# ethereum/pos-evolution

Hardware: AMD Instinct MI355X
Metric: attestations aggregated/sec + get_head() p50 latency at 1M validators (higher is better)
Workload: dtype int32

## Files before the change

pos_evolution_amd/csrc/att_bodies.inc:

```
#include <algorithm>
#include "att_row.h"
#include "kernels.h"
#include "wave64.h"

namespace posevo {

namespace {

constexpr uint32_t VAL_EQUIVOCATING_BIT = 0x04u;
constexpr uint32_t FLAG_SIG_VALID = 0x1u, FLAG_FROM_BLOCK = 0x2u, FLAG_OVERLAPPING = 0x4u;
constexpr int32_t ST_OK = 0, ST_EPOCH_TIME = 1, ST_EPOCH_SLOT = 2, ST_UNKNOWN_TARGET = 3, ST_UNKNOWN_BLOCK = 4,
                  ST_BLOCK_AFTER_SLOT = 5, ST_TARGET_NOT_ANCESTOR = 6, ST_SLOT_NOT_PAST = 7, ST_NO_TABLE = 8,
                  ST_INDEX_RANGE = 9, ST_BITS_LENGTH = 10, ST_EMPTY = 11, ST_BAD_SIGNATURE = 12, ST_INCLUSION = 13,
                  ST_SOURCE = 14;
constexpr uint32_t ERR_INVALID_ARG = 1, ERR_CAPACITY = 10, ERR_NO_COMMITTEES = 11;

struct Row9 { uint4 q[9]; };
__device__ __forceinline__ void load_row(Row9& r, const uint4* __restrict__ rows, uint32_t i)
{
    const uint4* p = rows + (size_t)9 * i;
#pragma unroll
    for (int k = 0; k < 9; ++k) r.q[k] = p[k];
}
__device__ __forceinline__ unsigned long long u64_of(uint32_t lo, uint32_t hi) { return ((unsigned long long)hi << 32) | lo; }
// ... 422 lines not shown
{
    uint32_t h = r0.x & bt.root_mask;
    for (;;) {
        const uint32_t idx = bt.root_tab[h];
        if (idx == NONE32) return NONE32;
        const uint4* q = reinterpret_cast<const uint4*>(bt.roots + 32ull * idx);
        if (same4(q[0], r0) && same4(q[1], r1)) return idx;
        h = (h + 1) & bt.root_mask;
    }
}
}

namespace {
__device__ __forceinline__ void att_validate_fc_body(const uint32_t g , const ValidateFcArgs& a)
{
    const uint4* __restrict__ rows = static_cast<const uint4*>(a.rows);
    const AttGroup* __restrict__ grp = a.grp;
    const AttPlan* __restrict__ plan = a.plan;
    const uint32_t cap = a.cap;
    const BlockTableDev& bt = a.bt;
    const FcCtx& fc = a.fc;
    const uint32_t* __restrict__ union_info = a.union_info;
    AttRow* __restrict__ out_rows = a.out_rows;
    int32_t* __restrict__ status_dev = a.status_dev;
    int32_t* __restrict__ status_host = a.status_host;
    uint32_t* __restrict__ count_host = a.count_host;
    uint32_t* __restrict__ err_host = a.err_host;
    const uint32_t ng = plan->n_groups;
    if (ng > cap) {
        if (g < ng) status_dev[g] = -1;
        if (g == 0) *err_host = ERR_CAPACITY;
        return;
    }
    if (g >= ng) return;
    const AttGroup G = grp[g];
    Row9 r;
    load_row(r, rows, G.rep);
    const unsigned long long slot = row_slot(r), tep = row_target_epoch(r), spe = fc.slots_per_epoch;
    const uint32_t flags = r.q[8].z;
    int32_t st = ST_OK;
    uint32_t blk = NONE32;
    if (!(flags & FLAG_FROM_BLOCK) && tep != fc.cur_epoch && tep != fc.prev_epoch) st = ST_EPOCH_TIME;
    else if (tep != slot / spe) st = ST_EPOCH_SLOT;
    else {
        const uint32_t tgt = find_block_dev(bt, r.q[6], r.q[7]);
        if (tgt == NONE32) st = ST_UNKNOWN_TARGET;
        else {
            blk = find_block_dev(bt, r.q[1], r.q[2]);
            if (blk == NONE32) st = ST_UNKNOWN_BLOCK;
            else {
                uint32_t p = bt.pos_of_idx[blk];
                if (bt.slot_pos[p] > slot) st = ST_BLOCK_AFTER_SLOT;
                else {
                    const unsigned long long start = tep * spe;
                    while (bt.slot_pos[p] > start && bt.parent_pos[p] != NONE32) p = bt.parent_pos[p];
                    if (p != bt.pos_of_idx[tgt]) st = ST_TARGET_NOT_ANCESTOR;
                    else if (fc.cur_slot < slot + 1) st = ST_SLOT_NOT_PAST;
                }
            }
        }
    }
    if (st == ST_OK && G.status_agg) st = (int32_t)G.status_agg;
    const uint32_t cnt = union_info[2 * g], overlap = union_info[2 * g + 1];
    if (st == ST_OK) {
        if (!G.sig_valid) st = ST_BAD_SIGNATURE;
        else if (overlap) st = ST_BAD_SIGNATURE;
        else if (cnt == 0) st = ST_EMPTY;
    }
    AttRow o;
    o.member_base = G.member_base;
    o.n_bits = G.size;
    o.bits_word = G.out_word;
    o.block_idx = blk;
    o.epoch_p1 = (uint32_t)tep + 1;
    o.order = g;
    o.flag_mask = 0;
    o.which = 0;
    o.slot = (uint32_t)slot;
    o.gate = g;
    out_rows[g] = o;
    status_dev[g] = st;
    status_host[g] = st;
    if (count_host) count_host[g] = st == ST_OK ? cnt : 0u;
}
}

namespace {
__device__ __forceinline__ void lmd_vm_tables_body(const unsigned long long v , const LmdVmArgs& a)
{
    const AttRow* __restrict__ rows = a.rows;
    const TablesDev& tables = a.tables;
    const uint32_t* __restrict__ cs0 = a.crow_start[0];
    const uint32_t* __restrict__ cs1 = a.crow_start[1];
    const uint32_t* __restrict__ cl0 = a.crow_list[0];
    const uint32_t* __restrict__ cl1 = a.crow_list[1];
    const AttPlan* __restrict__ plan = a.plan;
    const uint32_t* __restrict__ bit_arena = a.bit_arena;
    const uint8_t* __restrict__ flags = a.flags;
    unsigned long long* __restrict__ vote_key = reinterpret_cast<unsigned long long*>(a.vote_key);
    uint32_t* __restrict__ vote_block = a.vote_block;
    uint32_t* __restrict__ vote_slot = a.vote_slot;
    const uint32_t* __restrict__ gates = a.gates;
    if (v >= a.n_val) return;
    uint32_t best_e = 0, best_order = NONE32, new_block = NONE32, new_slot = 0;
    bool loaded = false;
    for (int t = 0; t < 2; ++t) {
        if (!tables.t[t].valid || plan->n_rows_table[t] == 0) continue;
        const uint32_t c = tables.t[t].inv_comm[v];
        if (c == NONE32) continue;
        const uint32_t* crow_start = t ? cs1 : cs0;
        const uint32_t* crow_list = t ? cl1 : cl0;
        const uint32_t kb = crow_start[c], ke = crow_start[c + 1];
        if (kb == ke) continue;
        if (!loaded) {
            if (flags[v] & VAL_EQUIVOCATING_BIT) return;
            best_e = (uint32_t)(vote_key[v] >> 32);
            loaded = true;
        }
        const uint32_t i = tables.t[t].inv_pos[v];
        for (uint32_t k = kb; k < ke; ++k) {
            const AttRow r = rows[crow_list[k]];
            if (i >= r.n_bits) continue;
            if (gates[r.gate] != 0) continue;
            if (!((bit_arena[r.bits_word + (i >> 5)] >> (i & 31)) & 1u)) continue;
            if (r.epoch_p1 > best_e || (r.epoch_p1 == best_e && new_block != NONE32 && r.order < best_order)) {
                best_e = r.epoch_p1;
                best_order = r.order;
                new_block = r.block_idx;
                new_slot = r.slot;
            }
        }
    }
    if (new_block != NONE32) {
        vote_key[v] = ((unsigned long long)best_e << 32) | 0xFFFFFFFFull;
        vote_block[v] = new_block;
        if (vote_slot) vote_slot[v] = new_slot;
    }
}
}

}
```

pos_evolution_amd/csrc/engine_internal.h:

```cpp
#pragma once
#include <hip/hip_runtime.h>
#include <dlfcn.h>
#include <rccl/rccl.h>

#include <algorithm>
#include <array>
#include <chrono>
#include <cstdlib>
#include <map>
#include <cstdio>
#include <cstddef>
#include <cstring>
#include <functional>
#include <memory>
#include <new>
#include <numeric>
#include <string>
#include <thread>
#include <unordered_map>
#include <vector>

#include "../../include/posevo.h"
#include "../../include/posevo_profile.h"
#include "att_row.h"
// ... 285 lines not shown
        hipEvent_t ev_leg = nullptr;
        bool leg_used = false;
        bool fenced = false, side_used = false, aux_used = false;
        bool fence_pending = false;
        bool aux_reads_scratch = false;
    };
    static constexpr int MAX_ARENAS = 16;
    int n_arenas = 3;
    PipeArena arena[MAX_ARENAS];
    int cur = 0;
    PipeArena& A() { return arena[cur]; }
    bool pipelining = false;
    uint64_t pipes_begun = 0, pipes_completed = 0;
    hipStream_t side_stream = nullptr;
    uint64_t arena_growths = 0;
    bool queues_distinct = false;
    hipStream_t fin_stream = nullptr;
    hipStream_t norm_stream = nullptr;
    hipEvent_t ev_tree = nullptr;
    hipStream_t g1_tail() const { return norm_stream ? norm_stream : fin_stream; }
    hipStream_t aux_stream = nullptr;
    hipStream_t aux_owned = nullptr;
    hipStream_t prep_stream = nullptr;
    DevBuf d_shuffle_scratch;
    hipStream_t sums_stream = nullptr;
    DevBuf d_sum_groups, d_sum_lane;
    uint32_t last_cmpl_groups = 0;
    hipEvent_t ev_aux_fork = nullptr;
    hipEvent_t ev_aux_switch = nullptr;
    static constexpr uint32_t STATE_ON_SIDE_MAX_ROWS = 1024;
    bool aux_busy = false;
    bool state_work_on_main = false;
    hipEvent_t ev_acc = nullptr;
    struct SigSeg {
        int arena;
        uint32_t n;
        bool compressed, check_subgroup;
        bool streaming;
        const uint8_t* d_in;
        const uint8_t* copy_from;
        size_t bytes;
        uint32_t* d_pts; int32_t* d_status;
        const UnionGroup* d_ug; const uint32_t* d_member_row; uint32_t ng_bound; const AttPlan* plan_dev;
        uint8_t* o_sig; uint32_t* o_bad; int32_t* o_st;
        uint32_t* keep_mont48; uint32_t* keep_bad;
    };
    std::vector<SigSeg> sig_batch;
    hipEvent_t ev_sig = nullptr;
    hipEvent_t ev_fork = nullptr, ev_join = nullptr;
    bool side_busy = false;
    bool side_ever = false;
    bool streaming = false;
    std::vector<std::function<int()>> deferred;
    struct HeldFc {
        bool active = false;
        int arena = -1;
        bool have_fc = false;
        bool have_head = false;
        ValidateFcArgs validate{};
        LmdVmArgs lmd{};
        VotesArgs votes{};
        TreeArgs tree{};
        std::function<int()> between;
        std::vector<std::function<int()>> g1;
        bool fence_pending = false;
    } held;
    bool pairing = std::getenv("POSEVO_PAIR") == nullptr || std::atoi(std::getenv("POSEVO_PAIR")) != 0;
    struct Tune {
        static int env(const char* name, int dflt)
        {
            const char* e = std::getenv(name);
            return e && *e ? std::atoi(e) : dflt;
        }
        int exclusive = env("POSEVO_ACC_EXCLUSIVE", 1);
        int state_on = env("POSEVO_STATE_ON", 2);
        int sig_batch = env("POSEVO_SIG_BATCH", 8);
        int queue_probe = env("POSEVO_QUEUE_PROBE", 1);
        int committee_sums = env("POSEVO_COMMITTEE_SUMS", 1);
        int g1_sparse = env("POSEVO_G1_SPARSE", 1);
        uint32_t g1_sparse_max() const
        {
            return g1_sparse <= 0 ? 0u : g1_sparse == 1 ? G1_SPARSE_MAX : std::min<uint32_t>((uint32_t)g1_sparse, G1_SPARSE_CAP);
        }
        uint32_t ssz_tile_log2 = (uint32_t)std::min<int>(SSZ_TILE_LOG2, std::max<int>(SSZ_TILE_LOG2_MIN, env("POSEVO_SSZ_TILE_LOG2", SSZ_TILE_LOG2)));
    } tune;

    struct ResGroup { uint32_t byte_off, n_bits, word, sig_valid, tag; };
    std::vector<ResGroup> res_groups;
    std::shared_ptr<std::vector<uint32_t>> res_info_host;
    bool res_valid = false;
    int res_arena = 0;
    uint64_t res_generation = 0;

    struct ResidentRows {
        bool valid = false;
        int arena = 0;
        uint32_t n_in = 0;
        const void* rows = nullptr;
        TablesDev tables{};
        uint64_t generation = 0;
        int set = 0;
        uint32_t n_groups = 0;
    } rr;

    int g1_tune_calls = 0;
    float g1_tune_best[2] = {1e30f, 1e30f};
    uint32_t g1_target_slots = 0;
    hipEvent_t g1_tune_ev[2] = {nullptr, nullptr};
    bool points30_valid = false;
    DevBuf d_points30, d_tmp_points30;

    ncclComm_t comm = nullptr, comm_g1 = nullptr;
    int early_rc = PE_OK;
    uint32_t xchg_blocks = 0;
    uint64_t xchg_nval = 0;
    bool last_agg_on_side = false;
    int dist_rank = 0, dist_world = 1;
    DevBuf d_xchg, d_xpart, d_xgather;
    pe_collectives coll{};
    bool coll_custom = false;
    bool dist_single_comm = false;
    bool dist_wedged = false;
    uint32_t dist_timeout_ms = 30000;
    uint32_t dist_max_groups = 0;
    hipEvent_t ev_xchg = nullptr;
    bool dist_ready() const { return comm != nullptr || coll_custom; }

    struct Slasher {
        bool enabled = false;
        uint32_t history = 0, max_data = 0;
        uint64_t n_val = 0;
        bool have_window = false;
        uint64_t window = 0;
        DevBuf d_rec, d_ids, d_counter, d_evidence;
        struct EpochData {
            std::vector<std::array<uint8_t, 128>> data;
            std::unordered_map<std::string, uint32_t> id_of;
        };
        std::vector<EpochData> epochs;
        bool on_device = false;
        uint32_t tab_size = 0;
        DevBuf d_data, d_count, d_tab;
        DevBuf d_work;
        std::vector<uint32_t> dev_count;
    } slasher;

    bool profiling = false;
    uint64_t acc_launches = 0;
    static constexpr uint32_t ACC_CLOCK_RING = 4096;
    unsigned long long* acc_clock = nullptr;
    uint64_t acc_clock_n = 0;
    KernelProfile prof[PE_KERNEL_COUNT];
    bool prof_timeline = false;
    bool prof_dominant_only = false;
    hipEvent_t prof_base = nullptr;
    struct TimelineEntry { int32_t kernel; float start_ms, dur_ms; };
    std::vector<TimelineEntry> prof_tl;
    std::vector<hipEvent_t> event_pool;
    HostTrace trace;
};

namespace posevo {

int fail(pe_engine* h, int code, const std::string& msg);
int hip_fail(pe_engine* h, hipError_t e, const char* what);
#define HIP_TRY(h, expr)                                        \
// ... 408 lines not shown
```

pos_evolution_amd/csrc/engine_resident.cpp:

```cpp
#include "engine_internal.h"


using namespace posevo;

namespace posevo {

namespace {

struct RrLayout {
    AttPlan* plan;
    uint32_t *slot_of, *rep_of, *gid_of_row, *ubytes, *member_row;
    PlanSync* sync;
    PlanRec* rec;
    AttGroup* grp;
    UnionGroup* ug;
    G1Group* g1;
    AttRow *rows_fc, *rows_st;
    int32_t *status_fc, *status_st;
    uint32_t* cmpl;
    uint32_t *crow_start[2], *crow_cursor[2], *crow_cnt[2], *crow_list[2];
    size_t bytes;
};

RrLayout rr_layout(uint8_t* base, uint32_t cap_n, uint32_t cap_c)
{
    RrLayout L;
    size_t off = 0;
    auto take = [&](size_t bytes) {
        uint8_t* p = base ? base + off : nullptr;
        off = (off + bytes + 255) & ~size_t(255);
        return p;
    };
    L.plan = reinterpret_cast<AttPlan*>(take(sizeof(AttPlan)));
    L.slot_of = reinterpret_cast<uint32_t*>(take(4ull * cap_n));
    L.rep_of = reinterpret_cast<uint32_t*>(take(4ull * cap_n));
    L.gid_of_row = reinterpret_cast<uint32_t*>(take(4ull * cap_n));
    L.sync = reinterpret_cast<PlanSync*>(take(sizeof(PlanSync)));
    L.rec = reinterpret_cast<PlanRec*>(take(sizeof(PlanRec) * ((size_t)cap_n / PLAN_WG + 1)));
    L.ubytes = reinterpret_cast<uint32_t*>(take(4ull * cap_n));
    L.member_row = reinterpret_cast<uint32_t*>(take(4ull * cap_n));
    L.grp = reinterpret_cast<AttGroup*>(take(sizeof(AttGroup) * (size_t)cap_n));
    L.ug = reinterpret_cast<UnionGroup*>(take(sizeof(UnionGroup) * (size_t)cap_n));
    L.g1 = reinterpret_cast<G1Group*>(take(sizeof(G1Group) * (size_t)cap_n));
    L.rows_fc = reinterpret_cast<AttRow*>(take(sizeof(AttRow) * (size_t)cap_n));
    L.rows_st = reinterpret_cast<AttRow*>(take(sizeof(AttRow) * (size_t)cap_n));
    L.status_fc = reinterpret_cast<int32_t*>(take(4ull * cap_n));
    L.status_st = reinterpret_cast<int32_t*>(take(4ull * cap_n));
    L.cmpl = reinterpret_cast<uint32_t*>(take(4ull * cap_n));
    for (int t = 0; t < 2; ++t) {
        L.crow_start[t] = reinterpret_cast<uint32_t*>(take(4ull * (cap_c + 1)));
        L.crow_cursor[t] = reinterpret_cast<uint32_t*>(take(4ull * (cap_c + 1)));
        L.crow_cnt[t] = reinterpret_cast<uint32_t*>(take(4ull * (cap_c + 1)));
        L.crow_list[t] = reinterpret_cast<uint32_t*>(take(4ull * cap_n));
    }
    L.bytes = off;
    return L;
}

struct RrSet {
    DevBuf &tab, &rr, &bits, &info;
    uint32_t &rows_cap, &comm_cap, &tab_size;
};
RrSet rr_set(pe_engine::PipeArena& a, int set)
{
    if (set == 0) return RrSet{a.d_rr_tab, a.d_rr, a.d_res_bits, a.d_res_info, a.rr_rows_cap, a.rr_comm_cap, a.rr_tab_size};
    return RrSet{a.x_rr_tab, a.x_rr, a.x_res_bits, a.x_res_info, a.x_rows_cap, a.x_comm_cap, a.x_tab_size};
}
RrLayout rr_of(pe_engine::PipeArena& a, int set = 0)
{
    const RrSet s = rr_set(a, set);
    return rr_layout(s.rr.as<uint8_t>(), s.rows_cap, s.comm_cap);
}

int rr_ensure(pe_engine* h, pe_engine::PipeArena& arena, int set, uint32_t n, uint32_t n_comm)
{
    {
        const RrSet rs = rr_set(arena, set);
        if (n <= rs.rows_cap && n_comm <= rs.comm_cap && rs.rr.p && rs.tab.p) return PE_OK;
    }
    PE_TRY(flush_pending(h));
    HIP_TRY(h, hipDeviceSynchronize());
    uint32_t cap_n = 1024, cap_c = 64;
    for (int i = 0; i < h->n_arenas; ++i) {
        const RrSet o = rr_set(h->arena[i], set);
        cap_n = std::max(cap_n, o.rows_cap);
        cap_c = std::max(cap_c, o.comm_cap);
    }
    while (cap_n < n) cap_n *= 2;
    while (cap_c < n_comm) cap_c *= 2;
    uint32_t tab = 2048;
    while (tab < 2 * cap_n) tab <<= 1;
    const RrLayout L = rr_layout(nullptr, cap_n, cap_c);
    for (int i = 0; i < h->n_arenas; ++i) {
        pe_engine::PipeArena& other = h->arena[i];
        if (set != 0 && &other != &arena) continue;
        const RrSet a = rr_set(other, set);
        if (cap_n <= a.rows_cap && cap_c <= a.comm_cap && a.rr.p && a.tab.p) continue;
        a.rr.release();
        a.tab.release();
        HIP_TRY(h, a.rr.ensure(L.bytes));
        HIP_TRY(h, a.tab.ensure(8ull * tab));
        HIP_TRY(h, hipMemsetAsync(a.tab.p, 0xFF, 4ull * tab, h->stream));
        HIP_TRY(h, hipMemsetAsync(a.tab.as<uint8_t>() + 4ull * tab, 0, 4ull * tab, h->stream));
        HIP_TRY(h, hipMemsetAsync(a.rr.p, 0, L.bytes, h->stream));
        a.rows_cap = cap_n;
        a.comm_cap = cap_c;
        a.tab_size = tab;
    }
    HIP_TRY(h, hipStreamSynchronize(h->stream));
    return PE_OK;
}

int candidate_tables(pe_engine* h, TablesDev* out, CommitteeTable* tabs[2])
{
    memset(out, 0, sizeof(*out));
    out->slots_per_epoch = h->cfg.slots_per_epoch;
    const uint64_t cur = epoch_at_slot(h, current_slot(h));
    const uint64_t prev = cur > 0 ? cur - 1 : cur;
    const uint64_t epochs[2] = {cur, prev};
    for (int k = 0; k < 2; ++k) {
        tabs[k] = nullptr;
        out->t[k].epoch = epochs[k];
        if (k == 1 && prev == cur) continue;
        CommitteeTable* t = find_table(h, epochs[k]);
        if (!t) continue;
        if (!t->is_partition || t->n_val_at_load != h->n_val || !t->d_inv_comm.p)
            return fail(h, PE_ERR_INVALID_ARG,
                        "rows in device memory: the committee tables of the current / previous epoch must partition the "
                        "registry they were loaded for (use host rows otherwise)");
        tabs[k] = t;
        out->t[k].members = t->d_members.as<uint32_t>();
        out->t[k].offsets = t->d_offsets.as<uint32_t>();
        out->t[k].inv_comm = t->d_inv_comm.as<uint32_t>();
        out->t[k].inv_pos = t->d_inv_pos.as<uint32_t>();
        out->t[k].n_committees = t->n_committees;
        out->t[k].valid = 1;
    }
    return PE_OK;
}

uint32_t g1_target_slots(const pe_engine* h)
{
    if (h->streaming) return G1_TARGET_LANES / 2;
    return h->g1_target_slots ? h->g1_target_slots : G1_TARGET_LANES;
}

}

int plan_error_to_status(pe_engine* h, uint32_t err, const char* who)
{
    switch (err) {
        case 0: return PE_OK;
        case 10: return fail(h, PE_ERR_CAPACITY, std::string(who) + ": output capacity too small for the groups formed");
        case 11: return fail(h, PE_ERR_NO_COMMITTEES, std::string(who) + ": no committee table for a group's target epoch");
        case 12: return fail(h, PE_ERR_NO_DEVICE, std::string(who) + ": a workgroup of k_att_plan gave up waiting for its predecessors' records");
        default:
            return fail(h, PE_ERR_INVALID_ARG, std::string(who) + ": a row was refused on the device (bits exceed the arena, "
                        "target epoch beyond 32 bits, committee index out of range or len(aggregation_bits) != len(committee))");
    }
}

MemKind mem_kind(const void* p)
{
    hipPointerAttribute_t pa;
    if (p && hipPointerGetAttributes(&pa, p) == hipSuccess)
        return pa.type == hipMemoryTypeDevice ? MemKind::Device : pa.type == hipMemoryTypeHost ? MemKind::Pinned : MemKind::Pageable;
    (void)hipGetLastError();
    return MemKind::Pageable;
}
bool rows_on_device(const void* p) { return p && p != (const void*)PE_ROWS_RESIDENT && mem_kind(p) == MemKind::Device; }

BlockTableDev block_table_dev(const pe_engine* h)
{
    BlockTableDev bt;
    bt.root_tab = h->d_broot_tab.as<uint32_t>();
    bt.root_mask = h->broot_mask;
    bt.roots = h->d_broots.as<uint8_t>();
    bt.slot_pos = h->d_bslot_pos.as<unsigned long long>();
    bt.parent_pos = h->d_tparent.as<uint32_t>();
    bt.pos_of_idx = h->d_tpos.as<uint32_t>();
    bt.n_blocks = (uint32_t)h->blocks.size();
    return bt;
}

int aggregate_resident(pe_engine* h, const pe_attestation* d_rows, uint32_t n, const uint8_t* bits_arena,
                       uint64_t arena_len, pe_attestation* out_atts, uint32_t* out_n_groups, uint32_t* group_of,
                       uint8_t* out_bits_arena, uint64_t out_arena_cap, uint8_t* out_aggpk96, uint32_t* out_count,
                       uint32_t* dev_partials, int set, const uint32_t* n_dev)
{
    if (!h->initialised) return fail(h, PE_ERR_STATE, "rows in device memory: the store's clock picks the committee tables; call pe_store_init first");
    if ((uintptr_t)d_rows & 15) return fail(h, PE_ERR_INVALID_ARG, "rows in device memory must be 16-byte aligned");
    if (arena_len >= 0xFFFFFFF0ull) return fail(h, PE_ERR_CAPACITY, "bit arena exceeds 4 GiB");
    if (n >= PLAN_MAX_ROWS) return fail(h, PE_ERR_CAPACITY, "rows in device memory: at most 2^24 - 1 rows per aggregate");
    const bool want_pk = out_aggpk96 != nullptr || dev_partials != nullptr;
    if (want_pk && !h->have_points) return fail(h, PE_ERR_STATE, "aggregate pubkeys requested but no pubkeys loaded");
    HostLap lap(&h->trace);
    TablesDev tables;
    CommitteeTable* tabs[2];
    PE_TRY(candidate_tables(h, &tables, tabs));
    const uint32_t n_comm = std::max(tables.t[0].n_committees, tables.t[1].n_committees);
    pe_engine::PipeArena& A = h->A();
    PE_TRY(rr_ensure(h, A, set, n, n_comm));
    const RrLayout L = rr_of(A, set);
    const RrSet RS = rr_set(A, set);
    const uint32_t target = g1_target_slots(h);
    const uint32_t slot_cap = std::max<uint32_t>(2 * G1_TARGET_LANES, (n + G1_WG - 1) / G1_WG * G1_WG);
    const size_t words_cap = (size_t)out_arena_cap / 4 + n + 16;
    Stage st(h);
    PE_TRY(st.reserve((size_t)arena_len + 256));
    const size_t pad_at = ((size_t)arena_len + 15) & ~size_t(15);
    const size_t off_arena = st.alloc(pad_at + 32);
    if (set == 0) {
        PE_TRY(ensure_quiesced_arenas(h, &pe_engine::PipeArena::d_res_bits, words_cap * 4 + 64));
        PE_TRY(ensure_quiesced_arenas(h, &pe_engine::PipeArena::d_res_info, 8ull * n + 64));
    } else {
        PE_TRY(ensure_quiesced(h, RS.bits, words_cap * 4 + 64));
        PE_TRY(ensure_quiesced(h, RS.info, 8ull * n + 64));
    }
    OutBlock ob(h);
    const size_t off_plan = ob.alloc(sizeof(AttPlan));
    const size_t off_rows = ob.alloc(sizeof(pe_attestation) * (size_t)n);
    const size_t off_gof = ob.alloc(4ull * n);
    const size_t off_obits = ob.alloc(words_cap * 4);
    const size_t off_oinfo = ob.alloc(8ull * n);
    const size_t off_opk = out_aggpk96 ? ob.alloc(96ull * n) : 0;
    G1Complement cm;
    bool by_cmpl = false;
    if (out_aggpk96 && !dev_partials && set == 0 && h->tune.committee_sums && !h->dist_ready())
        for (int t = 0; t < 2; ++t) {
            if (tabs[t]) PE_TRY(committee_sums_build_wanted(h, tabs[t]));
            if (tabs[t] && tabs[t]->sums_valid && tabs[t]->d_sums.p && tabs[t]->ev_sums) {
                cm.sums[t] = tabs[t]->d_sums.as<uint32_t>();
                cm.ev[t] = tabs[t]->ev_sums;
                by_cmpl = true;
            }
        }
    const size_t off_ocm = by_cmpl ? ob.alloc(4ull * n) : 0;
    PE_TRY(ob.ensure());
    if (by_cmpl) {
        cm.cmpl = L.cmpl;
        cm.info = RS.info.as<uint32_t>();
    }
    if (want_pk) {
        PE_TRY(ensure_quiesced_arenas(h, &pe_engine::PipeArena::d_partials, std::max<size_t>(PE_G1_PARTIAL_BYTES, (size_t)PE_G1_PARTIAL_BYTES * n)));
        PE_TRY(ensure_quiesced_arenas(h, &pe_engine::PipeArena::d_lane_partials, (size_t)G1_LANE_PARTIAL_BYTES * slot_cap));
        PE_TRY(ensure_quiesced(h, h->d_partials, std::max<size_t>(PE_G1_PARTIAL_BYTES, (size_t)PE_G1_PARTIAL_BYTES * n)));
        PE_TRY(ensure_quiesced(h, h->d_lane_partials, (size_t)G1_LANE_PARTIAL_BYTES * slot_cap));
    }
    lap.mark("ragg.1_reserve");
    *out_n_groups = 0;
    AttPlan* plan_host = ob.host<AttPlan>(off_plan);
    memset(plan_host, 0, sizeof(AttPlan));
    plan_host->error = 0xFFFFFFFFu;
    const MemKind arena_kind = arena_len ? mem_kind(bits_arena) : MemKind::Pageable;
    hipStream_t ms = h->stream;
    const bool pair_ok = h->held.active && h->held.arena != h->cur && set == 0 && !n_dev && hold_eligible(h);
    if (h->held.active && !pair_ok) PE_TRY(held_issue(h));
    if (set == 0) {
        if (!h->deferred.empty()) PE_TRY(run_deferred(h));
        if (A.side_used) HIP_TRY(h, hipStreamWaitEvent(ms, h->ev_join, 0));
        if (sig_batch_holds(h, h->cur)) PE_TRY(sig_batch_flush(h));
        if (A.leg_used) HIP_TRY(h, hipStreamWaitEvent(ms, A.ev_leg, 0));
        PE_TRY(aux_join(h, ms));
    }
    h->res_valid = false;
    h->rr.valid = false;
    const size_t deferred_before = h->deferred.size();
    struct Unwind {
        pe_engine* h; size_t keep; bool armed = true;
        ~Unwind() { if (armed) { h->rr.valid = false; if (h->deferred.size() > keep) h->deferred.resize(keep); } }
    } unwind{h, deferred_before};
    bool ingest_copies = false;
    if (arena_kind == MemKind::Pageable) {
        memcpy(st.host<uint8_t>(off_arena), bits_arena, arena_len);
        memset(st.host<uint8_t>(off_arena) + arena_len, 0, pad_at + 32 - arena_len);
        HIP_TRY(h, st.upload());
    } else if (arena_len) {
        if (arena_kind == MemKind::Device && (reinterpret_cast<uintptr_t>(bits_arena) & 15) == 0 && n > 0) ingest_copies = true;
        else HIP_TRY(h, hipMemcpyAsync(st.dev<uint8_t>(off_arena), bits_arena, arena_len,
                                       arena_kind == MemKind::Device ? hipMemcpyDeviceToDevice : hipMemcpyHostToDevice, ms));
    }
    lap.mark("ragg.2_bits");
    uint32_t* cnt_tab = RS.tab.as<uint32_t>() + RS.tab_size;
    const IngestArgs ia{d_rows, n, RS.tab.as<uint32_t>(), cnt_tab, RS.tab_size - 1, L.slot_of, arena_len, L.plan,
                        st.dev<uint8_t>(off_arena) + pad_at, n_dev, ingest_copies ? bits_arena : nullptr,
// ... 116 lines not shown
        if (out_aggpk96) memcpy(out_aggpk96, pin + off_opk, 96ull * ng);
        h->last_cmpl_groups = 0;
        if (by_cmpl) {
            const uint32_t* ocm = reinterpret_cast<const uint32_t*>(pin + off_ocm);
            for (uint32_t g = 0; g < ng; ++g) h->last_cmpl_groups += ocm[g] != NONE32 ? 1u : 0u;
        }
        return PE_OK;
    };
    HostLap lap2(&h->trace);
    const int rc = finish_call(h, st, ob, complete);
    lap2.mark("ragg.5_wait_outputs");
    return rc;
}

int resident_plan_dev(pe_engine* h, const AttPlan** out)
{
    if (!h->rr.valid) return fail(h, PE_ERR_STATE, "no aggregate over rows in device memory on this handle");
    *out = rr_of(h->arena[h->rr.arena], h->rr.set).plan;
    return PE_OK;
}

int resident_parts(pe_engine* h, ResidentParts* out)
{
    if (!h->rr.valid) return fail(h, PE_ERR_STATE, "no aggregate over rows in device memory on this handle");
    pe_engine::PipeArena& RA = h->arena[h->rr.arena];
    const RrLayout L = rr_of(RA, h->rr.set);
    const RrSet RS = rr_set(RA, h->rr.set);
    out->rows = h->rr.rows;
    out->grp = L.grp;
    out->plan = L.plan;
    out->res_bits = RS.bits.as<uint32_t>();
    out->res_info = RS.info.as<uint32_t>();
    out->n_in = h->rr.n_in;
    return PE_OK;
}

int resident_lists(pe_engine* h, const UnionGroup** ug, const uint32_t** member_row)
{
    if (!h->rr.valid) return fail(h, PE_ERR_STATE, "no aggregate over rows in device memory on this handle");
    const RrLayout L = rr_of(h->arena[h->rr.arena], h->rr.set);
    *ug = L.ug;
    *member_row = L.member_row;
    return PE_OK;
}

int resident_precheck(pe_engine* h, const char* who)
{
    if (!h->rr.valid) return fail(h, PE_ERR_STATE, std::string(who) + ": PE_ROWS_RESIDENT without a pe_aggregate over rows in device memory on this handle");
    TablesDev now;
    CommitteeTable* tabs[2];
    PE_TRY(candidate_tables(h, &now, tabs));
    for (int t = 0; t < 2; ++t)
        if (now.t[t].epoch != h->rr.tables.t[t].epoch || now.t[t].valid != h->rr.tables.t[t].valid ||
            now.t[t].members != h->rr.tables.t[t].members)
            return fail(h, PE_ERR_STATE, std::string(who) + ": the store's clock or its committee tables changed since the resident pe_aggregate: aggregate again");
    return PE_OK;
}

int on_attestation_resident(pe_engine* h, uint32_t cap, int32_t* status, uint32_t* out_count)
{
    PE_TRY(resident_precheck(h, "pe_on_attestation_batch"));
    if (cap == 0) return PE_OK;
    if (h->held.active && (h->held.arena != h->cur || h->held.have_fc || h->held.have_head)) PE_TRY(held_issue(h));
    HostLap lap(&h->trace);
    PE_TRY(refresh_tree(h));
    pe_engine::PipeArena& RA = h->arena[h->rr.arena];
    const RrLayout L = rr_of(RA, h->rr.set);
    const RrSet RS = rr_set(RA, h->rr.set);
    Stage st(h);
    OutBlock ob(h);
    const size_t off_status = ob.alloc(4ull * cap);
    const size_t off_count = ob.alloc(4ull * cap);
    const size_t off_err = ob.alloc(16);
    PE_TRY(ob.ensure());
    *ob.host<uint32_t>(off_err) = 0;
    FcCtx fc;
    fc.cur_slot = current_slot(h);
    fc.cur_epoch = epoch_at_slot(h, fc.cur_slot);
    fc.prev_epoch = fc.cur_epoch > 0 ? fc.cur_epoch - 1 : 0;
    fc.slots_per_epoch = h->cfg.slots_per_epoch;
    const uint32_t n_launch = std::max<uint32_t>(h->rr.n_in, 1);
    memset(ob.host<int32_t>(off_status), 0, 4ull * cap);
    memset(ob.host<uint32_t>(off_count), 0, 4ull * cap);
    const ValidateFcArgs va{h->rr.rows, L.grp, L.plan, n_launch, cap, block_table_dev(h), fc, RS.info.as<uint32_t>(), L.rows_fc,
                            L.status_fc, ob.host<int32_t>(off_status), ob.host<uint32_t>(off_count), ob.host<uint32_t>(off_err)};
    const LmdVmArgs la{L.rows_fc, h->rr.tables, {L.crow_start[0], L.crow_start[1]}, {L.crow_list[0], L.crow_list[1]}, L.plan,
                       RS.bits.as<uint32_t>(), h->d_flags.as<uint8_t>(), h->n_val, h->d_vote_key.as<uint64_t>(),
                       h->d_vote_block.as<uint32_t>(), h->cfg.vote_expiry_slots ? h->d_vote_slot.as<uint32_t>() : nullptr,
                       reinterpret_cast<const uint32_t*>(L.status_fc)};
    if (hold_eligible(h) && h->rr.arena == h->cur && h->rr.set == 0 && h->n_val) {
        h->held.validate = va;
        h->held.lmd = la;
        h->held.have_fc = true;
        h->held.active = true;
        h->held.arena = h->cur;
    } else {
        if (h->held.active) PE_TRY(held_issue(h));
        {
            ProfScope ps(h, PE_KERNEL_ATT_VALIDATE);
            launch_att_validate_fc(h->stream, va);
        }
        ProfScope ps(h, PE_KERNEL_LMD);
        launch_lmd_vm_tables(h->stream, la);
    }
    HIP_TRY(h, hipGetLastError());
    lap.mark("ratt.1_launch");
    const size_t base = ob.base;
    const int ai = h->cur;
    auto complete = [h, ai, base, off_status, off_count, off_err, cap, status, out_count]() -> int {
        const uint8_t* pin = h->arena[ai].h_pin.as<uint8_t>() + base;
        const uint32_t err = *reinterpret_cast<const uint32_t*>(pin + off_err);
        if (err) return plan_error_to_status(h, err, "pe_on_attestation_batch (PE_ROWS_RESIDENT)");
        memcpy(status, pin + off_status, 4ull * cap);
        if (out_count) memcpy(out_count, pin + off_count, 4ull * cap);
        return PE_OK;
    };
    HostLap lap2(&h->trace);
    const int rc = finish_call(h, st, ob, complete);
    lap2.mark("ratt.2_wait_outputs");
    return rc;
}

int process_attestation_resident(pe_engine* h, const pe_state_ctx* sc, uint32_t cap, int32_t* status, uint64_t* out_numerators)
{
    PE_TRY(resident_precheck(h, "pe_process_attestation_batch"));
    if (cap == 0) return PE_OK;
    const uint64_t spe = h->cfg.slots_per_epoch;
    if (spe > 64) return fail(h, PE_ERR_CAPACITY, "PE_ROWS_RESIDENT: SLOTS_PER_EPOCH above 64");
    uint32_t tip;
    if (!find_block(h, to_root(sc->chain_tip_root), &tip)) return fail(h, PE_ERR_UNKNOWN_ROOT, "chain tip unknown");
    HostLap lap(&h->trace);
    PE_TRY(refresh_tree(h));
    pe_engine::PipeArena& RA = h->arena[h->rr.arena];
    const RrLayout L = rr_of(RA, h->rr.set);
    const RrSet RS = rr_set(RA, h->rr.set);
    Stage st(h);
    StateCtxDev S;
    memset(&S, 0, sizeof(S));
    S.slot = sc->slot;
    S.cur_epoch = sc->slot / spe;
    S.prev_epoch = S.cur_epoch > 0 ? S.cur_epoch - 1 : 0;
    S.slots_per_epoch = spe;
    S.min_inclusion_delay = h->cfg.min_attestation_inclusion_delay;
    S.sqrt_spe = isqrt64(spe);
    S.cj_epoch = sc->current_justified_epoch;
    S.pj_epoch = sc->previous_justified_epoch;
    memcpy(S.cj_root, sc->current_justified_root, 32);
    memcpy(S.pj_root, sc->previous_justified_root, 32);
    S.base_reward_per_increment = sc->base_reward_per_increment;
    {
        uint32_t cur = tip;
        for (uint64_t j = spe; j-- > 0;) {
            if (S.slot + j < spe) { S.head_blk[j] = NONE32; continue; }
            cur = get_ancestor(h, cur, S.slot + j - spe);
            S.head_blk[j] = cur;
        }
        S.tgt_blk[0] = get_ancestor(h, tip, S.cur_epoch * spe);
        S.tgt_blk[1] = get_ancestor(h, tip, S.prev_epoch * spe);
    }
    OutBlock ob(h);
    const size_t off_err = ob.alloc(16);
    const size_t off_status = ob.alloc(4ull * cap);
    const size_t off_num = ob.alloc(8ull * cap);
    PE_TRY(ob.ensure());
    *ob.host<uint32_t>(off_err) = 0;
    memset(ob.host<int32_t>(off_status), 0, 4ull * cap);
    memset(ob.host<uint64_t>(off_num), 0, 8ull * cap);
    const uint32_t n_launch = std::max<uint32_t>(h->rr.n_in, 1);
    hipStream_t ss = state_stream_begin(h, true, n_launch);
    {
        ProfScope ps(h, PE_KERNEL_ATT_VALIDATE, ss);
        launch_att_validate_state(ss, h->rr.rows, L.grp, L.plan, n_launch, cap, block_table_dev(h), S,
// ... 30 lines not shown
```

pos_evolution_amd/csrc/kernels.h:

```cpp
#pragma once
#include <hip/hip_runtime.h>
#include <stdint.h>

namespace posevo {

template <int TAG>
static bool first_use_on_this_device()
{
    static bool done[64] = {false};
    int dev = 0;
    (void)hipGetDevice(&dev);
    if (dev < 0 || dev >= 64) return true;
    if (done[dev]) return false;
    done[dev] = true;
    return true;
}

constexpr uint32_t NONE32 = 0xFFFFFFFFu;
constexpr int G1_ROW_WORDS = 32;
constexpr int G2_WG_SLOTS = 128;
constexpr int G1_WG = 256;
constexpr int G1_LANE_PARTIAL_BYTES = 208;
constexpr int TREE_MAX_BLOCKS = 8192;
constexpr int VOTES_MAX_WG = 256;
// ... 107 lines not shown
    uint32_t last_error;
    unsigned long long total_members;
};
struct AttGroup {
    uint32_t rep;
    uint32_t n_atts, list_start, cursor;
    uint32_t n_bits, out_word, out_byte;
    uint32_t table;
    uint32_t pos, size, member_base;
    uint32_t sig_valid;
    uint32_t status_agg;
    uint32_t index_over;
    uint32_t pad[2];
};
struct BlockTableDev {
    const uint32_t* root_tab;
    uint32_t root_mask;
    const uint8_t* roots;
    const unsigned long long* slot_pos;
    const uint32_t* parent_pos;
    const uint32_t* pos_of_idx;
    uint32_t n_blocks;
};
struct FcCtx {
    unsigned long long cur_slot, cur_epoch, prev_epoch, slots_per_epoch;
};
struct StateCtxDev {
    unsigned long long slot, cur_epoch, prev_epoch, slots_per_epoch, min_inclusion_delay, sqrt_spe;
    unsigned long long cj_epoch, pj_epoch;
    uint8_t cj_root[32], pj_root[32];
    uint32_t tgt_blk[2];
    uint32_t head_blk[64];
    unsigned long long base_reward_per_increment;
};
struct PlanSync {
    uint32_t ticket;
    uint32_t max_size;
    uint32_t rows_t[2];
    uint32_t mis_key;
    uint32_t err;
    uint32_t pad[2];
    unsigned long long total_members, pad2[3];
};
struct PlanRec {
    unsigned long long agg[3], incl[3], pad[2];
};
constexpr uint32_t PLAN_WG = 256;
constexpr uint32_t PLAN_MAX_ROWS = 1u << 24;
struct AttPlanArgs {
    const void* rows; uint32_t n; const uint32_t* n_dev;
    const uint32_t* tab; const uint32_t* cnt_tab; const uint32_t* slot_of;
    uint32_t* rep_of; uint32_t* gid_of_row;
    AttGroup* grp; UnionGroup* ug;
    uint32_t* crow_start[2]; uint32_t* crow_cursor[2]; uint32_t* crow_cnt[2];
    PlanSync* sync; PlanRec* rec;
    AttPlan* plan; AttPlan* plan_host;
    uint64_t out_arena_cap; uint32_t target_slots, slot_cap, min_k, want_pk;
    TablesDev tables;
};
void launch_att_plan(hipStream_t s, const AttPlanArgs& a);
void launch_att_pack(hipStream_t s, const void* rows, const AttGroup* grp, const AttPlan* plan, const uint32_t* res_bits,
                     const uint32_t* res_info, uint32_t slots, uint32_t wps, uint32_t* send);
void launch_att_unpack(hipStream_t s, const uint32_t* recv, uint32_t world, uint32_t slots, uint32_t wps, void* out_rows,
                       uint32_t* out_bits, uint32_t* n_dev, uint32_t* err_host);
void launch_att_validate_state(hipStream_t s, const void* rows, const AttGroup* grp, const AttPlan* plan, uint32_t n_bound,
                               uint32_t cap, BlockTableDev bt, const StateCtxDev& st, const uint32_t* union_info,
                               AttRow* out_rows, int32_t* status_dev, int32_t* status_host, uint32_t* err_host);
void launch_participation_tables(hipStream_t s, const AttRow* rows, TablesDev tables, uint32_t* const crow_start[2],
                                 uint32_t* const crow_list[2], const AttPlan* plan, const uint32_t* bit_arena,
                                 const uint16_t* eff_increments, uint64_t base_reward_per_increment,
                                 uint32_t* part_cur_words, uint32_t* part_prev_words, uint64_t* numerators,
                                 const uint32_t* gates, uint32_t cap);

struct IngestArgs {
    const void* rows; uint32_t n;
    uint32_t* tab; uint32_t* cnt_tab;
    uint32_t tab_mask;
    uint32_t* slot_of;
    uint64_t arena_len; AttPlan* plan;
    void* arena_pad32;
    const uint32_t* n_dev;
    const void* arena_src; void* arena_dst;
};
struct ValidateFcArgs {
    const void* rows; const AttGroup* grp; const AttPlan* plan;
    uint32_t n_bound, cap;
    BlockTableDev bt; FcCtx fc;
    const uint32_t* union_info; AttRow* out_rows; int32_t* status_dev; int32_t* status_host; uint32_t* count_host;
    uint32_t* err_host;
};
struct LmdVmArgs {
    const AttRow* rows; TablesDev tables; const uint32_t* crow_start[2]; const uint32_t* crow_list[2];
    const AttPlan* plan; const uint32_t* bit_arena; const uint8_t* flags; uint64_t n_val; uint64_t* vote_key;
    uint32_t* vote_block; uint32_t* vote_slot; const uint32_t* gates;
};
struct MembersArgs {
    const void* rows; uint32_t n; uint32_t* tab; uint32_t* cnt_tab; const uint32_t* slot_of; const uint32_t* rep_of;
    const uint32_t* gid_of_row; AttGroup* grp; AttPlan* plan; uint32_t* ubytes; uint32_t* member_row;
    uint32_t* host_group_of; void* host_out_rows; const uint32_t* n_dev;
    G1Group* g1; uint32_t* crow_cursor[2]; uint32_t* crow_list[2];
};
struct VotesArgs {
    const uint32_t* vote_block; const uint64_t* eff_balance; const uint8_t* flags; uint64_t n_val;
    uint32_t filter_slashed; const uint32_t* pos_of_idx; uint32_t n_blocks; uint64_t* direct; VoteTotals* totals;
    const uint32_t* vote_slot; uint32_t min_vote_slot;
};
struct UnionArgs {
    const UnionGroup* groups; uint32_t n_groups; const uint32_t* att_bytes;
    const uint8_t* bit_arena;
    uint32_t* out_arena;
    uint32_t* out_info;
    uint32_t* host_arena; uint32_t* host_info;
    const AttPlan* plan_dev;
    uint32_t* cmpl; uint32_t* host_cmpl; const AttGroup* grp; uint32_t sums_ok[2];
};
struct TreeArgs {
    TreeDev tree; uint64_t* direct; const VoteTotals* totals; uint64_t ov_balance, ov_num; int use_override;
    uint32_t justified_pos, boost_pos; uint64_t slots_per_epoch, boost_percent, balance_increment;
    uint64_t* weights_by_idx; uint32_t* head_idx; int clear_direct;
};
struct RemapArgs {
    uint32_t* vote_block; uint64_t n_val;
    const uint32_t* map; uint32_t n_old;
    unsigned long long* counts;
};
constexpr uint32_t VOTE_PRUNED = 0xFFFFFFFEu;
constexpr int REMAP_WG = 256;
constexpr unsigned REMAP_MAX_WG = 256;
void launch_votes_remap(hipStream_t s, const RemapArgs& a);
void launch_att_ingest(hipStream_t s, const IngestArgs& a);
void launch_att_validate_fc(hipStream_t s, const ValidateFcArgs& a);
void launch_lmd_vm_tables(hipStream_t s, const LmdVmArgs& a);
void launch_att_members(hipStream_t s, const MembersArgs& a);
void launch_votes(hipStream_t s, const VotesArgs& a, int lean);
void votes_clear_exchange(hipStream_t s, uint64_t* direct, uint32_t n_blocks, VoteTotals* totals);
void launch_bits_union(hipStream_t s, const UnionArgs& a);
void launch_tree(hipStream_t s, const TreeArgs& a, int lean);
bool launch_pair_ingest_validate(hipStream_t s, const IngestArgs& rows_next, const ValidateFcArgs& fc_prev);
bool launch_pair_plan_lmd(hipStream_t s, const AttPlanArgs& rows_next, const LmdVmArgs& fc_prev);
bool launch_pair_members_votes(hipStream_t s, const MembersArgs& rows_next, const VotesArgs& fc_prev);
bool launch_pair_union_tree(hipStream_t s, const UnionArgs& rows_next, const TreeArgs& fc_prev);
void pair_kernels_preload();

struct SlashRow {
    uint32_t bits_byte;
    uint32_t n_bits;
    uint32_t source, target;
    uint32_t id;
    uint32_t pad[3];
};
struct SlashTable {
    const uint32_t* inv_comm;
    const uint32_t* inv_pos;
    const uint32_t* crow_start;
};
struct SlashArgs {
    const SlashRow* rows;
    const SlashTable* tables; uint32_t n_tables;
    const uint32_t* crow_list;
    const uint8_t* bits;
    unsigned long long* rec; uint32_t* ids; uint32_t history; uint64_t n_val;
    uint32_t* counter;
    uint32_t* evidence; uint32_t cap;
    uint8_t* flags;
};
constexpr int SLASH_NV = 4;
void launch_slash_scan(hipStream_t s, const SlashArgs& a);

struct SlashRowsArgs {
    const void* rows;
    const AttGroup* grp; uint32_t n_groups;
    uint64_t window; uint32_t history;
    uint32_t max_data, tab_mask;
    uint32_t slot_of_table[2];
    uint8_t* data; uint32_t* count; uint32_t* tab;
    int32_t* status;
    uint32_t* err;
// ... 212 lines not shown
```

Measured before the change: 6.425 billion.

## Add per-committee LMD digest to skip row-list indirection in vote update

The validate kernel now writes, for each committee whose row list holds a single attestation, a 32-byte digest with that row's fields plus a generation stamp, or a MULTI marker when the list has several rows. The per-validator LMD kernel first loads the digests for both tables and, in the single-row case, applies the vote directly, avoiding the crow_start/crow_list/row indirection chain. It falls back to walking the list for multi-row committees. The change adds digest storage, stamp wraparound handling that resets digests with a full device sync, and extra loads issued unconditionally when digests are enabled.

```diff
diff --git a/pos_evolution_amd/csrc/att_bodies.inc b/pos_evolution_amd/csrc/att_bodies.inc
--- a/pos_evolution_amd/csrc/att_bodies.inc
+++ b/pos_evolution_amd/csrc/att_bodies.inc
@@ -528,18 +528,46 @@
     status_dev[g] = st;
     status_host[g] = st;
     if (count_host) count_host[g] = st == ST_OK ? cnt : 0u;
+    if (a.digest[0] && G.status_agg == (uint32_t)ST_OK) {
+        const uint32_t* __restrict__ cs = G.table ? a.crow_start[1] : a.crow_start[0];
+        uint4* d = reinterpret_cast<uint4*>((G.table ? a.digest[1] : a.digest[0]) + G.pos);
+        if (cs[G.pos + 1] - cs[G.pos] == 1) {
+            d[0] = make_uint4(a.stamp, o.n_bits, o.bits_word, o.block_idx);
+            d[1] = make_uint4(o.epoch_p1, o.order, o.slot, o.gate);
+        } else
+            *reinterpret_cast<uint2*>(d) = make_uint2(a.stamp, LMD_DIGEST_MULTI);
+    }
 }
 }
 
 namespace {
+struct LmdBest { uint32_t e, order, block, slot; };
+__device__ __forceinline__ void lmd_offer(LmdBest& b, uint32_t epoch_p1, uint32_t order, uint32_t block_idx, uint32_t slot)
+{
+    if (epoch_p1 > b.e || (epoch_p1 == b.e && b.block != NONE32 && order < b.order)) {
+        b.e = epoch_p1;
+        b.order = order;
+        b.block = block_idx;
+        b.slot = slot;
+    }
+}
+__device__ __forceinline__ void lmd_walk_list(LmdBest& b, const AttRow* __restrict__ rows, const uint32_t* __restrict__ crow_start,
+                                              const uint32_t* __restrict__ crow_list, const uint32_t c, const uint32_t i,
+                                              const uint32_t* __restrict__ gates, const uint32_t* __restrict__ bit_arena)
+{
+    const uint32_t kb = crow_start[c], ke = crow_start[c + 1];
+    for (uint32_t k = kb; k < ke; ++k) {
+        const AttRow r = rows[crow_list[k]];
+        if (i >= r.n_bits) continue;
+        if (gates[r.gate] != 0) continue;
+        if (!((bit_arena[r.bits_word + (i >> 5)] >> (i & 31)) & 1u)) continue;
+        lmd_offer(b, r.epoch_p1, r.order, r.block_idx, r.slot);
+    }
+}
 __device__ __forceinline__ void lmd_vm_tables_body(const unsigned long long v , const LmdVmArgs& a)
 {
     const AttRow* __restrict__ rows = a.rows;
     const TablesDev& tables = a.tables;
-    const uint32_t* __restrict__ cs0 = a.crow_start[0];
-    const uint32_t* __restrict__ cs1 = a.crow_start[1];
-    const uint32_t* __restrict__ cl0 = a.crow_list[0];
-    const uint32_t* __restrict__ cl1 = a.crow_list[1];
     const AttPlan* __restrict__ plan = a.plan;
     const uint32_t* __restrict__ bit_arena = a.bit_arena;
     const uint8_t* __restrict__ flags = a.flags;
@@ -548,41 +576,46 @@
     uint32_t* __restrict__ vote_slot = a.vote_slot;
     const uint32_t* __restrict__ gates = a.gates;
     if (v >= a.n_val) return;
-    uint32_t best_e = 0, best_order = NONE32, new_block = NONE32, new_slot = 0;
-    bool loaded = false;
-    for (int t = 0; t < 2; ++t) {
-        if (!tables.t[t].valid || plan->n_rows_table[t] == 0) continue;
-        const uint32_t c = tables.t[t].inv_comm[v];
-        if (c == NONE32) continue;
-        const uint32_t* crow_start = t ? cs1 : cs0;
-        const uint32_t* crow_list = t ? cl1 : cl0;
-        const uint32_t kb = crow_start[c], ke = crow_start[c + 1];
-        if (kb == ke) continue;
-        if (!loaded) {
-            if (flags[v] & VAL_EQUIVOCATING_BIT) return;
-            best_e = (uint32_t)(vote_key[v] >> 32);
-            loaded = true;
-        }
-        const uint32_t i = tables.t[t].inv_pos[v];
-        for (uint32_t k = kb; k < ke; ++k) {
-            const AttRow r = rows[crow_list[k]];
-            if (i >= r.n_bits) continue;
-            if (gates[r.gate] != 0) continue;
-            if (!((bit_arena[r.bits_word + (i >> 5)] >> (i & 31)) & 1u)) continue;
-            if (r.epoch_p1 > best_e || (r.epoch_p1 == best_e && new_block != NONE32 && r.order < best_order)) {
-                best_e = r.epoch_p1;
-                best_order = r.order;
-                new_block = r.block_idx;
-                new_slot = r.slot;
-            }
-        }
-    }
-    if (new_block != NONE32) {
-        vote_key[v] = ((unsigned long long)best_e << 32) | 0xFFFFFFFFull;
-        vote_block[v] = new_block;
-        if (vote_slot) vote_slot[v] = new_slot;
-    }
-}
-}
-
-}
+    const bool v0 = tables.t[0].valid != 0, v1 = tables.t[1].valid != 0;
+    uint32_t nr0 = plan->n_rows_table[0], nr1 = plan->n_rows_table[1];
+    uint32_t c0 = v0 ? tables.t[0].inv_comm[v] : NONE32, c1 = v1 ? tables.t[1].inv_comm[v] : NONE32;
+    uint32_t i0 = v0 ? tables.t[0].inv_pos[v] : 0u, i1 = v1 ? tables.t[1].inv_pos[v] : 0u;
+    uint32_t fl = flags[v];
+    unsigned long long key = vote_key[v];
+    asm volatile("" : "+v"(nr0), "+v"(nr1), "+v"(c0), "+v"(c1), "+v"(i0), "+v"(i1), "+v"(fl), "+v"(key));
+    const bool use0 = v0 && nr0 != 0 && c0 != NONE32 && !(fl & VAL_EQUIVOCATING_BIT);
+    const bool use1 = v1 && nr1 != 0 && c1 != NONE32 && !(fl & VAL_EQUIVOCATING_BIT);
+    const bool digests = a.digest[0] != nullptr;
+    uint4 d0a = make_uint4(0, 0, 0, 0), d0b = d0a, d1a = d0a, d1b = d0a;
+    if (digests) {
+        const uint4* p0 = reinterpret_cast<const uint4*>(a.digest[0] + (use0 ? c0 : 0u));
+        const uint4* p1 = reinterpret_cast<const uint4*>(a.digest[1] + (use1 ? c1 : 0u));
+        d0a = p0[0]; d0b = p0[1]; d1a = p1[0]; d1b = p1[1];
+        asm volatile("" : "+v"(d0a.x), "+v"(d0a.y), "+v"(d0a.z), "+v"(d0a.w), "+v"(d0b.x), "+v"(d0b.y), "+v"(d0b.z), "+v"(d0b.w),
+                          "+v"(d1a.x), "+v"(d1a.y), "+v"(d1a.z), "+v"(d1a.w), "+v"(d1b.x), "+v"(d1b.y), "+v"(d1b.z), "+v"(d1b.w));
+    }
+    const bool live0 = use0 && (!digests || d0a.x == a.stamp), live1 = use1 && (!digests || d1a.x == a.stamp);
+    const bool one0 = digests && live0 && d0a.y != LMD_DIGEST_MULTI, one1 = digests && live1 && d1a.y != LMD_DIGEST_MULTI;
+    const bool hit0 = one0 && i0 < d0a.y, hit1 = one1 && i1 < d1a.y;
+    uint32_t g0 = 0, g1 = 0, w0 = 0, w1 = 0;
+    if (digests) {
+        g0 = gates[hit0 ? d0b.w : 0u];
+        g1 = gates[hit1 ? d1b.w : 0u];
+        w0 = bit_arena[hit0 ? d0a.z + (i0 >> 5) : 0u];
+        w1 = bit_arena[hit1 ? d1a.z + (i1 >> 5) : 0u];
+        asm volatile("" : "+v"(g0), "+v"(g1), "+v"(w0), "+v"(w1));
+    }
+    LmdBest b{(uint32_t)(key >> 32), NONE32, NONE32, 0u};
+    if (hit0 && g0 == 0 && ((w0 >> (i0 & 31)) & 1u)) lmd_offer(b, d0b.x, d0b.y, d0a.w, d0b.z);
+    else if (live0 && !one0) lmd_walk_list(b, rows, a.crow_start[0], a.crow_list[0], c0, i0, gates, bit_arena);
+    if (hit1 && g1 == 0 && ((w1 >> (i1 & 31)) & 1u)) lmd_offer(b, d1b.x, d1b.y, d1a.w, d1b.z);
+    else if (live1 && !one1) lmd_walk_list(b, rows, a.crow_start[1], a.crow_list[1], c1, i1, gates, bit_arena);
+    if (b.block != NONE32) {
+        vote_key[v] = ((unsigned long long)b.e << 32) | 0xFFFFFFFFull;
+        vote_block[v] = b.block;
+        if (vote_slot) vote_slot[v] = b.slot;
+    }
+}
+}
+
+}
diff --git a/pos_evolution_amd/csrc/engine_internal.h b/pos_evolution_amd/csrc/engine_internal.h
--- a/pos_evolution_amd/csrc/engine_internal.h
+++ b/pos_evolution_amd/csrc/engine_internal.h
@@ -391,6 +391,7 @@
         {
             return g1_sparse <= 0 ? 0u : g1_sparse == 1 ? G1_SPARSE_MAX : std::min<uint32_t>((uint32_t)g1_sparse, G1_SPARSE_CAP);
         }
+        int lmd_digest = env("POSEVO_LMD_DIGEST", 1);
         uint32_t ssz_tile_log2 = (uint32_t)std::min<int>(SSZ_TILE_LOG2, std::max<int>(SSZ_TILE_LOG2_MIN, env("POSEVO_SSZ_TILE_LOG2", SSZ_TILE_LOG2)));
     } tune;
 
diff --git a/pos_evolution_amd/csrc/engine_resident.cpp b/pos_evolution_amd/csrc/engine_resident.cpp
--- a/pos_evolution_amd/csrc/engine_resident.cpp
+++ b/pos_evolution_amd/csrc/engine_resident.cpp
@@ -19,6 +19,7 @@
     int32_t *status_fc, *status_st;
     uint32_t* cmpl;
     uint32_t *crow_start[2], *crow_cursor[2], *crow_cnt[2], *crow_list[2];
+    LmdDigest* digest[2];
     size_t bytes;
 };
 
@@ -52,6 +53,7 @@
         L.crow_cursor[t] = reinterpret_cast<uint32_t*>(take(4ull * (cap_c + 1)));
         L.crow_cnt[t] = reinterpret_cast<uint32_t*>(take(4ull * (cap_c + 1)));
         L.crow_list[t] = reinterpret_cast<uint32_t*>(take(4ull * cap_n));
+        L.digest[t] = reinterpret_cast<LmdDigest*>(take(sizeof(LmdDigest) * ((size_t)cap_c + 1)));
     }
     L.bytes = off;
     return L;
@@ -107,6 +109,23 @@
         a.comm_cap = cap_c;
         a.tab_size = tab;
     }
+    HIP_TRY(h, hipStreamSynchronize(h->stream));
+    return PE_OK;
+}
+
+uint32_t digest_stamp(uint64_t generation) { return (uint32_t)(generation % 0xFFFFFFFFull) + 1u; }
+int digest_stamps_wrap(pe_engine* h)
+{
+    PE_TRY(flush_pending(h));
+    HIP_TRY(h, hipDeviceSynchronize());
+    for (int i = 0; i < h->n_arenas; ++i)
+        for (int set = 0; set < 2; ++set) {
+            const RrSet rs = rr_set(h->arena[i], set);
+            if (!rs.rr.p) continue;
+            const RrLayout L = rr_layout(rs.rr.as<uint8_t>(), rs.rows_cap, rs.comm_cap);
+            for (int t = 0; t < 2; ++t)
+                HIP_TRY(h, hipMemsetAsync(L.digest[t], 0, sizeof(LmdDigest) * ((size_t)rs.comm_cap + 1), h->stream));
+        }
     HIP_TRY(h, hipStreamSynchronize(h->stream));
     return PE_OK;
 }
@@ -201,6 +220,7 @@
     const uint32_t n_comm = std::max(tables.t[0].n_committees, tables.t[1].n_committees);
     pe_engine::PipeArena& A = h->A();
     PE_TRY(rr_ensure(h, A, set, n, n_comm));
+    if (h->tune.lmd_digest && (h->rr.generation + 1) % 0xFFFFFFFFull == 0) PE_TRY(digest_stamps_wrap(h));
     const RrLayout L = rr_of(A, set);
     const RrSet RS = rr_set(A, set);
     const uint32_t target = g1_target_slots(h);
@@ -483,12 +503,16 @@
     const uint32_t n_launch = std::max<uint32_t>(h->rr.n_in, 1);
     memset(ob.host<int32_t>(off_status), 0, 4ull * cap);
     memset(ob.host<uint32_t>(off_count), 0, 4ull * cap);
+    const bool dg = h->tune.lmd_digest != 0;
+    const uint32_t stamp = digest_stamp(h->rr.generation);
     const ValidateFcArgs va{h->rr.rows, L.grp, L.plan, n_launch, cap, block_table_dev(h), fc, RS.info.as<uint32_t>(), L.rows_fc,
-                            L.status_fc, ob.host<int32_t>(off_status), ob.host<uint32_t>(off_count), ob.host<uint32_t>(off_err)};
+                            L.status_fc, ob.host<int32_t>(off_status), ob.host<uint32_t>(off_count), ob.host<uint32_t>(off_err),
+                            {L.crow_start[0], L.crow_start[1]}, {dg ? L.digest[0] : nullptr, dg ? L.digest[1] : nullptr}, stamp};
     const LmdVmArgs la{L.rows_fc, h->rr.tables, {L.crow_start[0], L.crow_start[1]}, {L.crow_list[0], L.crow_list[1]}, L.plan,
                        RS.bits.as<uint32_t>(), h->d_flags.as<uint8_t>(), h->n_val, h->d_vote_key.as<uint64_t>(),
                        h->d_vote_block.as<uint32_t>(), h->cfg.vote_expiry_slots ? h->d_vote_slot.as<uint32_t>() : nullptr,
-                       reinterpret_cast<const uint32_t*>(L.status_fc)};
+                       reinterpret_cast<const uint32_t*>(L.status_fc),
+                       {dg ? L.digest[0] : nullptr, dg ? L.digest[1] : nullptr}, stamp};
     if (hold_eligible(h) && h->rr.arena == h->cur && h->rr.set == 0 && h->n_val) {
         h->held.validate = va;
         h->held.lmd = la;
diff --git a/pos_evolution_amd/csrc/kernels.h b/pos_evolution_amd/csrc/kernels.h
--- a/pos_evolution_amd/csrc/kernels.h
+++ b/pos_evolution_amd/csrc/kernels.h
@@ -213,17 +213,26 @@
     const uint32_t* n_dev;
     const void* arena_src; void* arena_dst;
 };
+struct alignas(32) LmdDigest {
+    uint32_t stamp;
+    uint32_t n_bits;
+    uint32_t bits_word, block_idx, epoch_p1, order, slot, gate;
+};
+static_assert(sizeof(LmdDigest) == 32, "one aligned 32-byte record");
+constexpr uint32_t LMD_DIGEST_MULTI = 0xFFFFFFFFu;
 struct ValidateFcArgs {
     const void* rows; const AttGroup* grp; const AttPlan* plan;
     uint32_t n_bound, cap;
     BlockTableDev bt; FcCtx fc;
     const uint32_t* union_info; AttRow* out_rows; int32_t* status_dev; int32_t* status_host; uint32_t* count_host;
     uint32_t* err_host;
+    const uint32_t* crow_start[2]; LmdDigest* digest[2]; uint32_t stamp;
 };
 struct LmdVmArgs {
     const AttRow* rows; TablesDev tables; const uint32_t* crow_start[2]; const uint32_t* crow_list[2];
     const AttPlan* plan; const uint32_t* bit_arena; const uint8_t* flags; uint64_t n_val; uint64_t* vote_key;
     uint32_t* vote_block; uint32_t* vote_slot; const uint32_t* gates;
+    const LmdDigest* digest[2]; uint32_t stamp;
 };
 struct MembersArgs {
     const void* rows; uint32_t n; uint32_t* tab; uint32_t* cnt_tab; const uint32_t* slot_of; const uint32_t* rep_of;
```

Result: slower. 5.801 billion (-9.7%).
